# fnzhan/EMLight

Hardware: AMD Instinct MI355X
Metric: training images/sec (regression step: DenseNet-BC fwd + Sinkhorn loss + bwd + Adam) (higher is better)
Workload: dtype f32; 1 GPU; RegressionNetwork train step, BASELINE configs[1]; per_gpu_batch=64, global_batch=64, anchors=128, parallelism=single

## Files before the change

### emlight_amd/csrc/dense_bwd.hip

```cpp
#include "eml_common.h"
#include "eml_dropout.h"

#include <cstdint>
#include <cstdlib>
#include <type_traits>

namespace {

using eml::f32x4;
using eml::f4c;
using eml::mfma16;
using eml::shfl_xor_d;

constexpr int kTH = 8, kTW = 32, kHH = kTH + 2, kHW = kTW + 2;

constexpr int kPSG = 14;
constexpr int kBD = 512;
constexpr int kGRows = 2;
constexpr int kGPass = kHH / kGRows;

template <bool FUSE, bool WIDE, bool DROP = false>
__global__ __launch_bounds__(kBD, 2) void conv3x3_bwd_data_kernel(
    const float* __restrict__ G, int ldg, int c0, const float* __restrict__ W2, const float* __restrict__ Z,
    const float* __restrict__ zmean, const float* __restrict__ zistd, float* __restrict__ DZ, int B, int H, int W,
// ... 1221 lines not shown
          const float4 is = *reinterpret_cast<const float4*>(istd + k4);
          float l1[4] = {0.f, 0.f, 0.f, 0.f}, l2[4] = {0.f, 0.f, 0.f, 0.f};
#pragma unroll
          for (int m = 0; m < 4; ++m) {
            if (p0 + 16 * m + r < P) {
              const float da[4] = {acc[m][n][0], acc[m][n][1], acc[m][n][2], acc[m][n][3]};
              constexpr int NSUB = POOL ? 4 : 1;
#pragma unroll
              for (int sub = 0; sub < NSUB; ++sub) {
                const size_t pi = pin[m] + (sub >> 1) * (size_t)Win + (sub & 1);
                const float4 xv = *reinterpret_cast<const float4*>(X + pi * ldx + k4);
                float4* gp = reinterpret_cast<float4*>(Gd + pi * ldg + k4);
                float4 g = accumulate ? *gp : make_float4(0.f, 0.f, 0.f, 0.f);
                const float f = POOL ? 0.25f : 1.0f;
                const float d0 = (fmaf(xv.x, sk.x, tk.x) > 0.f) ? f * da[0] : 0.f;
                const float d1 = (fmaf(xv.y, sk.y, tk.y) > 0.f) ? f * da[1] : 0.f;
                const float d2 = (fmaf(xv.z, sk.z, tk.z) > 0.f) ? f * da[2] : 0.f;
                const float d3 = (fmaf(xv.w, sk.w, tk.w) > 0.f) ? f * da[3] : 0.f;
                g.x = fmaf(sk.x, d0, g.x);
                g.y = fmaf(sk.y, d1, g.y);
                g.z = fmaf(sk.z, d2, g.z);
                g.w = fmaf(sk.w, d3, g.w);
                *gp = g;
                l1[0] += d0;
                l1[1] += d1;
                l1[2] += d2;
                l1[3] += d3;
                l2[0] = fmaf(d0, (xv.x - mu.x) * is.x, l2[0]);
                l2[1] = fmaf(d1, (xv.y - mu.y) * is.y, l2[1]);
                l2[2] = fmaf(d2, (xv.z - mu.z) * is.z, l2[2]);
                l2[3] = fmaf(d3, (xv.w - mu.w) * is.w, l2[3]);
              }
            }
          }
#pragma unroll
          for (int g = 0; g < 4; ++g) {
            l1[g] = eml::row16_sum(l1[g]);
            l2[g] = eml::row16_sum(l2[g]);
            if (r == 0) {
              my[2 * (k4 + g)] += (double)l1[g];
              my[2 * (k4 + g) + 1] += (double)l2[g];
            }
          }
        }
      }
    }
  }
  __syncthreads();
  for (int e = tid; e < Kp * 2; e += 256)
    partials[(size_t)blockIdx.x * Kp * 2 + e] =
        (sacc[e] + sacc[(size_t)Kp * 2 + e]) + (sacc[(size_t)2 * Kp * 2 + e] + sacc[(size_t)3 * Kp * 2 + e]);
}

template <int MT, int NCH, bool ACC , bool MASKED = false, int NJO = 0>
__global__ __launch_bounds__(256, 2) void transition_bwd_data_kernel(
    const float* __restrict__ DY, int ld_dy, const float* __restrict__ Zr, int ld_z, const float* __restrict__ cA,
    const float* __restrict__ cB, const float* __restrict__ cC, int Ko, const float* __restrict__ Wd,
    const float* __restrict__ X, int ldx, const float* __restrict__ scale1, const float* __restrict__ shift1,
    const float* __restrict__ mean, const float* __restrict__ istd, int P, int Hin, int Win, int Kp,
    float* __restrict__ Gd, int ldg, double* __restrict__ partials ,
    const unsigned short* __restrict__ mask16) {
  extern __shared__ __attribute__((aligned(16))) float smem[];
  double* sacc = reinterpret_cast<double*>(smem);
  float* vec_l = reinterpret_cast<float*>(sacc + (size_t)4 * Kp * 2);
  float* co_l = vec_l + 4 * Kp;
  float* stg = co_l + 3 * Ko + (size_t)(threadIdx.x >> 6) * 16 * 36;
  const int tid = threadIdx.x, lane = tid & 63, wave = tid >> 6;
  const int r = lane & 15, kk = lane >> 4;
  for (int e = tid; e < 4 * Kp * 2; e += 256) sacc[e] = 0.0;
  for (int e = tid; e < Kp; e += 256) {
    vec_l[e] = scale1[e];
    vec_l[Kp + e] = shift1[e];
    vec_l[2 * Kp + e] = MASKED ? 0.f : mean[e];
    vec_l[3 * Kp + e] = MASKED ? 0.f : istd[e];
  }
  for (int e = tid; e < Ko; e += 256) {
    co_l[e] = cA[e];
    co_l[Ko + e] = cB[e];
    co_l[2 * Ko + e] = cC[e];
  }
  __syncthreads();
  double* my = sacc + (size_t)wave * Kp * 2;
  const int nnt = Kp >> 4, njo = Ko >> 4;
  constexpr int TP = 64 * MT;
  const int ntiles = (P + TP - 1) / TP;
  const int Wo = Win >> 1, Ho = Hin >> 1;

  for (int tile = blockIdx.x; tile < ntiles; tile += gridDim.x) {
    const int p0 = tile * TP + wave * 16 * MT;
    long prow[MT];
    size_t pin[MT];
    bool pv[MT];
#pragma unroll
    for (int m = 0; m < MT; ++m) {
      pv[m] = p0 + 16 * m + r < P;
      prow[m] = min(p0 + 16 * m + r, P - 1);
      const int b = (int)(prow[m] / (Ho * Wo)), rem = (int)(prow[m] - (long)b * (Ho * Wo));
      const int oy = rem / Wo, ox = rem - oy * Wo;
      pin[m] = (size_t)(b * Hin + 2 * oy) * Win + 2 * ox;
    }
    size_t pinx[MT][2];
    bool pvx[MT][2];
    if constexpr (MASKED && !ACC) {
#pragma unroll
      for (int m = 0; m < MT; ++m)
#pragma unroll
        for (int h = 0; h < 2; ++h) {
// ... 89 lines not shown
            dz[m].y = fmaf(a4.y, ry[m].y, fmaf(b4.y, rz[m].y, c4.y));
            dz[m].z = fmaf(a4.z, ry[m].z, fmaf(b4.z, rz[m].z, c4.z));
            dz[m].w = fmaf(a4.w, ry[m].w, fmaf(b4.w, rz[m].w, c4.w));
          }
          group_step(jo, dz);
        }
      }
      if constexpr (MASKED && !ACC) {
        float l1n[NCH][4];
        float4 skn[NCH];
#pragma unroll
        for (int n = 0; n < NCH; ++n) {
          skn[n] = *reinterpret_cast<const float4*>(vec_l + 16 * min(nt0 + n, nnt - 1) + 4 * kk);
#pragma unroll
          for (int g = 0; g < 4; ++g) l1n[n][g] = 0.f;
        }
        const int piece = lane & 7;
        const bool col_ok = nt0 + (piece >> 2) < nnt;
#pragma unroll
        for (int m = 0; m < MT; ++m) {
#pragma unroll
          for (int sub = 0; sub < 4; ++sub) {
#pragma unroll
            for (int n = 0; n < NCH; ++n) {
              const unsigned b = pv[m] ? mk[m][n] >> (4 * sub) : 0u;
              const float d0 = (b & 1u) ? 0.25f * acc[m][n][0] : 0.f, d1 = (b & 2u) ? 0.25f * acc[m][n][1] : 0.f;
              const float d2 = (b & 4u) ? 0.25f * acc[m][n][2] : 0.f, d3 = (b & 8u) ? 0.25f * acc[m][n][3] : 0.f;
              *reinterpret_cast<f32x4*>(stg + r * 36 + 16 * n + 4 * kk) = f32x4{skn[n].x * d0, skn[n].y * d1, skn[n].z * d2, skn[n].w * d3};
              if (nt0 + n < nnt) {
                l1n[n][0] += d0;
                l1n[n][1] += d1;
                l1n[n][2] += d2;
                l1n[n][3] += d3;
              }
            }
            __builtin_amdgcn_fence(__ATOMIC_RELEASE, "wavefront");
            __builtin_amdgcn_wave_barrier();
            __builtin_amdgcn_fence(__ATOMIC_ACQUIRE, "wavefront");
            const size_t suboff = ((size_t)(sub >> 1) * Win + (sub & 1)) * (size_t)ldg + 16 * nt0 + 4 * piece;
#pragma unroll
            for (int h = 0; h < 2; ++h) {
              const f32x4 v = *reinterpret_cast<const f32x4*>(stg + ((lane >> 3) + 8 * h) * 36 + 4 * piece);
              if (pvx[m][h] && col_ok) *reinterpret_cast<f32x4*>(Gd + pinx[m][h] * ldg + suboff) = v;
            }
            __builtin_amdgcn_fence(__ATOMIC_RELEASE, "wavefront");
            __builtin_amdgcn_wave_barrier();
            __builtin_amdgcn_fence(__ATOMIC_ACQUIRE, "wavefront");
          }
        }
#pragma unroll
        for (int n = 0; n < NCH; ++n) {
          if (nt0 + n < nnt) {
            const int k4 = 16 * (nt0 + n) + 4 * kk;
#pragma unroll
            for (int g = 0; g < 4; ++g) {
              const float t1 = eml::row16_sum(l1n[n][g]);
              if (r == 0) my[2 * (k4 + g)] += (double)t1;
            }
          }
        }
      } else {
#pragma unroll
      for (int n = 0; n < NCH; ++n) {
        const int nt = nt0 + n;
        if (nt < nnt) {
          const int k4 = 16 * nt + 4 * kk;
          const float4 sk = *reinterpret_cast<const float4*>(vec_l + k4);
          const float4 tk = *reinterpret_cast<const float4*>(vec_l + Kp + k4);
          const float4 mu = *reinterpret_cast<const float4*>(vec_l + 2 * Kp + k4);
          const float4 is = *reinterpret_cast<const float4*>(vec_l + 3 * Kp + k4);
          float l1[4] = {0.f, 0.f, 0.f, 0.f}, l2[4] = {0.f, 0.f, 0.f, 0.f};
#pragma unroll
          for (int m = 0; m < MT; ++m) {
            const float da0 = 0.25f * acc[m][n][0], da1 = 0.25f * acc[m][n][1];
            const float da2 = 0.25f * acc[m][n][2], da3 = 0.25f * acc[m][n][3];
#pragma unroll
            for (int sub = 0; sub < 4; ++sub) {
              float4 g = make_float4(0.f, 0.f, 0.f, 0.f);
              if constexpr (ACC) g = gs[m][n][sub];
              float d0, d1, d2, d3;
              float4 x = make_float4(0.f, 0.f, 0.f, 0.f);
              if constexpr (MASKED) {
                const unsigned b = pv[m] ? mk[m][n] >> (4 * sub) : 0u;
                d0 = (b & 1u) ? da0 : 0.f;
                d1 = (b & 2u) ? da1 : 0.f;
                d2 = (b & 4u) ? da2 : 0.f;
                d3 = (b & 8u) ? da3 : 0.f;
              } else {
                x = xv[m][n][sub];
                d0 = (pv[m] && fmaf(x.x, sk.x, tk.x) > 0.f) ? da0 : 0.f;
                d1 = (pv[m] && fmaf(x.y, sk.y, tk.y) > 0.f) ? da1 : 0.f;
                d2 = (pv[m] && fmaf(x.z, sk.z, tk.z) > 0.f) ? da2 : 0.f;
                d3 = (pv[m] && fmaf(x.w, sk.w, tk.w) > 0.f) ? da3 : 0.f;
              }
              g.x = fmaf(sk.x, d0, g.x);
              g.y = fmaf(sk.y, d1, g.y);
              g.z = fmaf(sk.z, d2, g.z);
              g.w = fmaf(sk.w, d3, g.w);
              if (pv[m]) {
                const size_t pi = pin[m] + (sub >> 1) * (size_t)Win + (sub & 1);
                *reinterpret_cast<float4*>(Gd + pi * ldg + k4) = g;
              }
              l1[0] += d0;
              l1[1] += d1;
              l1[2] += d2;
              l1[3] += d3;
              if constexpr (!MASKED) {
                l2[0] = fmaf(d0, (x.x - mu.x) * is.x, l2[0]);
                l2[1] = fmaf(d1, (x.y - mu.y) * is.y, l2[1]);
                l2[2] = fmaf(d2, (x.z - mu.z) * is.z, l2[2]);
                l2[3] = fmaf(d3, (x.w - mu.w) * is.w, l2[3]);
              }
            }
          }
#pragma unroll
          for (int g = 0; g < 4; ++g) {
            l1[g] = eml::row16_sum(l1[g]);
            if constexpr (!MASKED) l2[g] = eml::row16_sum(l2[g]);
            if (r == 0) {
              my[2 * (k4 + g)] += (double)l1[g];
              if constexpr (!MASKED) my[2 * (k4 + g) + 1] += (double)l2[g];
            }
          }
        }
      }
      }
    }
  }
  __syncthreads();
  for (int e = tid; e < Kp * 2; e += 256)
    partials[(size_t)blockIdx.x * Kp * 2 + e] =
        (sacc[e] + sacc[(size_t)Kp * 2 + e]) + (sacc[(size_t)2 * Kp * 2 + e] + sacc[(size_t)3 * Kp * 2 + e]);
}

struct BwdLayer {
  const float* DZ;
  const float* Zr;
  const float* cA;
  const float* cB;
  const float* cC;
  const float* Wd;
  const float* scale1;
  const float* shift1;
  double* partials;
  int Kp;
};

template <int NL, int MT , bool RAW = false ,
          bool MASKED = false, bool TOP = false>
__global__ __launch_bounds__(256, 2) void conv1x1_bwd_data_multi_kernel(BwdLayer L0, BwdLayer L1,
                                                                        const float* __restrict__ X, int ldx,
                                                                        const float* __restrict__ mean,
                                                                        const float* __restrict__ istd, int P,
                                                                        int k_lo, int k_hi, float* __restrict__ Gd,
                                                                        int ldg, int KpMax,
                                                                        const unsigned long long* __restrict__ M0,
                                                                        const unsigned long long* __restrict__ M1,
                                                                        float* __restrict__ Top) {
  extern __shared__ __attribute__((aligned(16))) float smem[];
  double* sacc = reinterpret_cast<double*>(smem);
  float* vec_l = reinterpret_cast<float*>(sacc + (size_t)NL * 4 * KpMax * 2);
  const int tid = threadIdx.x, lane = tid & 63, wave = tid >> 6;
  const int r = lane & 15, kk = lane >> 4;
  const BwdLayer Ls[2] = {L0, L1};
  for (int e = tid; e < NL * 4 * KpMax * 2; e += 256) sacc[e] = 0.0;
  for (int e = tid; e < KpMax; e += 256) {
    vec_l[e] = MASKED ? 0.f : mean[e];
    vec_l[KpMax + e] = MASKED ? 0.f : istd[e];
#pragma unroll
    for (int j = 0; j < NL; ++j) {
      vec_l[(2 + 2 * j) * KpMax + e] = e < Ls[j].Kp ? Ls[j].scale1[e] : 0.f;
      vec_l[(3 + 2 * j) * KpMax + e] = e < Ls[j].Kp ? Ls[j].shift1[e] : 0.f;
    }
  }
  __syncthreads();
  constexpr int TP = 64 * MT;
  const int ntiles = (P + TP - 1) / TP;
  const int nt_lo = k_lo >> 4, nt_hi = (k_hi + 15) >> 4;
  constexpr int NCH = 2;

  float4 wq[2][3][NCH];
  auto load_w = [&](int j, int nt0, float4 (&dst)[3][NCH]) {
    const int nnt = Ls[j].Kp >> 4;
#pragma unroll
    for (int jo = 0; jo < 3; ++jo)
#pragma unroll
      for (int n = 0; n < NCH; ++n) {
        const int nt = min(nt0 + n, nnt - 1);
        dst[jo][n] = *reinterpret_cast<const float4*>(Ls[j].Wd + ((((size_t)nt * 3 + jo) * 4 + kk) * 16 + r) * 4);
      }
  };
  load_w(0, nt_lo, wq[0]);
  int wsel = 0;

  for (int tile = blockIdx.x; tile < ntiles; tile += gridDim.x) {
    const int p0 = tile * TP + wave * 16 * MT;
    long prow[MT];
    bool pv[MT];
#pragma unroll
    for (int m = 0; m < MT; ++m) {
      pv[m] = p0 + 16 * m + r < P;
      prow[m] = min(p0 + 16 * m + r, P - 1);
    }
    unsigned long long pvb[MT];
#pragma unroll
    for (int m = 0; m < MT; ++m) pvb[m] = MASKED ? __ballot(pv[m]) : 0ull;
    float4 dz[NL][3][MT];
#pragma unroll
    for (int j = 0; j < NL; ++j)
#pragma unroll
      for (int jo = 0; jo < 3; ++jo) {
        const int ch = 16 * jo + 4 * kk;
        if constexpr (RAW) {
#pragma unroll
          for (int m = 0; m < MT; ++m) dz[j][jo][m] = *reinterpret_cast<const float4*>(Ls[j].DZ + prow[m] * 48 + ch);
        } else {
          const float4 a4 = *reinterpret_cast<const float4*>(Ls[j].cA + ch);
          const float4 b4 = *reinterpret_cast<const float4*>(Ls[j].cB + ch);
          const float4 c4 = *reinterpret_cast<const float4*>(Ls[j].cC + ch);
#pragma unroll
          for (int m = 0; m < MT; ++m) {
            const float4 dy = *reinterpret_cast<const float4*>(Ls[j].DZ + prow[m] * 48 + ch);
            const float4 zr = *reinterpret_cast<const float4*>(Ls[j].Zr + prow[m] * 48 + ch);
            dz[j][jo][m].x = fmaf(a4.x, dy.x, fmaf(b4.x, zr.x, c4.x));
            dz[j][jo][m].y = fmaf(a4.y, dy.y, fmaf(b4.y, zr.y, c4.y));
            dz[j][jo][m].z = fmaf(a4.z, dy.z, fmaf(b4.z, zr.z, c4.z));
            dz[j][jo][m].w = fmaf(a4.w, dy.w, fmaf(b4.w, zr.w, c4.w));
          }
        }
      }
    for (int nt0 = nt_lo; nt0 < nt_hi; nt0 += NCH) {
      float4 gs[MT][NCH], xv[MT][NCH];
#pragma unroll
      for (int n = 0; n < NCH; ++n) {
        const int k4 = 16 * min(nt0 + n, nt_hi - 1) + 4 * kk;
        const int k4l = (k4 + 3 >= k_lo && k4 < k_hi) ? k4 : (k_lo & ~3);
#pragma unroll
        for (int m = 0; m < MT; ++m) {
          gs[m][n] = *reinterpret_cast<const float4*>(Gd + prow[m] * ldg + k4l);
          if constexpr (!MASKED) xv[m][n] = *reinterpret_cast<const float4*>(X + prow[m] * ldx + k4l);
        }
      }
      const int nt_next = nt0 + NCH < nt_hi ? nt0 + NCH : nt_lo;
#pragma unroll
      for (int j = 0; j < NL; ++j) {
        const int nnt = Ls[j].Kp >> 4;
        unsigned long long mk[MT][NCH][4];
        if constexpr (MASKED) {
          const unsigned long long* __restrict__ Mj = j == 0 ? M0 : M1;
#pragma unroll
          for (int m = 0; m < MT; ++m)
#pragma unroll
            for (int n = 0; n < NCH; ++n) {
              const size_t wi =
                  ((size_t)__builtin_amdgcn_readfirstlane((p0 >> 4) + m) * nnt + min(nt0 + n, nnt - 1)) * 4;
#pragma unroll
              for (int g = 0; g < 4; ++g) mk[m][n][g] = Mj[wi + g];
            }
        }
        const int cur = NL == 2 ? j : wsel;
        if (j + 1 < NL)
          load_w(j + 1, nt0, wq[cur ^ 1]);
        else
          load_w(0, nt_next, wq[cur ^ 1]);
        __builtin_amdgcn_sched_barrier(0);
        f32x4 acc[MT][NCH];
#pragma unroll
        for (int m = 0; m < MT; ++m)
#pragma unroll
          for (int n = 0; n < NCH; ++n) acc[m][n] = f32x4{0.f, 0.f, 0.f, 0.f};
#pragma unroll
        for (int jo = 0; jo < 3; ++jo)
#pragma unroll
          for (int t = 0; t < 4; ++t)
#pragma unroll
            for (int n = 0; n < NCH; ++n)
#pragma unroll
              for (int m = 0; m < MT; ++m) acc[m][n] = mfma16(f4c(wq[cur][jo][n], t), f4c(dz[j][jo][m], t), acc[m][n]);
        if (NL == 1) wsel ^= 1;
        double* my = sacc + ((size_t)(j * 4 + wave) * KpMax) * 2;
#pragma unroll
        for (int n = 0; n < NCH; ++n) {
          const int nt = nt0 + n;
          if (nt < nnt && nt < nt_hi) {
            const int k4 = 16 * nt + 4 * kk;
            const float4 mu = *reinterpret_cast<const float4*>(vec_l + k4);
            const float4 is = *reinterpret_cast<const float4*>(vec_l + KpMax + k4);
            const float4 sk = *reinterpret_cast<const float4*>(vec_l + (2 + 2 * j) * KpMax + k4);
            const float4 tk = *reinterpret_cast<const float4*>(vec_l + (3 + 2 * j) * KpMax + k4);
            const bool in0 = k4 + 0 >= k_lo && k4 + 0 < k_hi, in1 = k4 + 1 >= k_lo && k4 + 1 < k_hi;
            const bool in2 = k4 + 2 >= k_lo && k4 + 2 < k_hi, in3 = k4 + 3 >= k_lo && k4 + 3 < k_hi;
            unsigned long long inb[4] = {0ull, 0ull, 0ull, 0ull};
            if constexpr (MASKED) {
              inb[0] = __ballot(in0);
              inb[1] = __ballot(in1);
              inb[2] = __ballot(in2);
              inb[3] = __ballot(in3);
            }
            float l1[4] = {0.f, 0.f, 0.f, 0.f}, l2[4] = {0.f, 0.f, 0.f, 0.f};
#pragma unroll
            for (int m = 0; m < MT; ++m) {
              float d0, d1, d2, d3;
              if constexpr (MASKED) {
                d0 = __builtin_amdgcn_inverse_ballot_w64(mk[m][n][0] & pvb[m] & inb[0]) ? acc[m][n][0] : 0.f;
                d1 = __builtin_amdgcn_inverse_ballot_w64(mk[m][n][1] & pvb[m] & inb[1]) ? acc[m][n][1] : 0.f;
                d2 = __builtin_amdgcn_inverse_ballot_w64(mk[m][n][2] & pvb[m] & inb[2]) ? acc[m][n][2] : 0.f;
                d3 = __builtin_amdgcn_inverse_ballot_w64(mk[m][n][3] & pvb[m] & inb[3]) ? acc[m][n][3] : 0.f;
              } else {
                const float4 x = xv[m][n];
                d0 = (pv[m] && in0 && fmaf(x.x, sk.x, tk.x) > 0.f) ? acc[m][n][0] : 0.f;
                d1 = (pv[m] && in1 && fmaf(x.y, sk.y, tk.y) > 0.f) ? acc[m][n][1] : 0.f;
                d2 = (pv[m] && in2 && fmaf(x.z, sk.z, tk.z) > 0.f) ? acc[m][n][2] : 0.f;
                d3 = (pv[m] && in3 && fmaf(x.w, sk.w, tk.w) > 0.f) ? acc[m][n][3] : 0.f;
                l2[0] = fmaf(d0, (x.x - mu.x) * is.x, l2[0]);
                l2[1] = fmaf(d1, (x.y - mu.y) * is.y, l2[1]);
                l2[2] = fmaf(d2, (x.z - mu.z) * is.z, l2[2]);
                l2[3] = fmaf(d3, (x.w - mu.w) * is.w, l2[3]);
              }
              gs[m][n].x = fmaf(sk.x, d0, gs[m][n].x);
              gs[m][n].y = fmaf(sk.y, d1, gs[m][n].y);
              gs[m][n].z = fmaf(sk.z, d2, gs[m][n].z);
              gs[m][n].w = fmaf(sk.w, d3, gs[m][n].w);
              l1[0] += d0;
              l1[1] += d1;
              l1[2] += d2;
              l1[3] += d3;
            }
#pragma unroll
            for (int g = 0; g < 4; ++g) {
              l1[g] = eml::row16_sum(l1[g]);
              if constexpr (!MASKED) l2[g] = eml::row16_sum(l2[g]);
              if (r == 0) {
                my[2 * (k4 + g)] += (double)l1[g];
                if constexpr (!MASKED) my[2 * (k4 + g) + 1] += (double)l2[g];
              }
            }
          }
        }
      }
#pragma unroll
      for (int n = 0; n < NCH; ++n) {
        const int nt = nt0 + n;
        if (nt < nt_hi) {
          const int k4 = 16 * nt + 4 * kk;
          const bool act = k4 + 3 >= k_lo && k4 < k_hi;
          if constexpr (TOP) {
            const int t = k4 - (k_hi - 24);
            float* cdst = Top + (t >= 12 ? (size_t)P * 12 + (t - 12) : (size_t)max(t, 0));
#pragma unroll
            for (int m = 0; m < MT; ++m) {
              float* dst = t >= 0 ? cdst + prow[m] * 12 : Gd + prow[m] * ldg + k4;
              if (pv[m] && act) *reinterpret_cast<float4*>(dst) = gs[m][n];
            }
          } else {
#pragma unroll
            for (int m = 0; m < MT; ++m) {
              if (pv[m] && act) *reinterpret_cast<float4*>(Gd + prow[m] * ldg + k4) = gs[m][n];
            }
          }
        }
      }
    }
  }
  __syncthreads();
#pragma unroll
  for (int j = 0; j < NL; ++j) {
    const int Kp = Ls[j].Kp;
    const double* base = sacc + (size_t)j * 4 * KpMax * 2;
    for (int e = tid; e < Kp * 2; e += 256)
      Ls[j].partials[(size_t)blockIdx.x * Kp * 2 + e] = (base[e] + base[(size_t)KpMax * 2 + e]) +
                                                        (base[(size_t)2 * KpMax * 2 + e] + base[(size_t)3 * KpMax * 2 + e]);
  }
}

template <int MT>
__global__ __launch_bounds__(256, 2) void conv1x1_bwd_narrow_kernel(
    const float* __restrict__ DZ, const float* __restrict__ W1 , int Cin, int k_lo,
    const float* __restrict__ X, int ldx, const float* __restrict__ scale1, const float* __restrict__ shift1,
    const float* __restrict__ mean, const float* __restrict__ istd, int P, const float* __restrict__ Gd, int ldg,
    float* __restrict__ N12, double* __restrict__ partials , int Kp) {
  __shared__ double red[4][12][2];
  const int tid = threadIdx.x, lane = tid & 63, wave = tid >> 6;
  const int r = lane & 15, kk = lane >> 4;
  float aw[3][4];
#pragma unroll
  for (int jo = 0; jo < 3; ++jo)
#pragma unroll
    for (int t = 0; t < 4; ++t) aw[jo][t] = r < 12 ? W1[(size_t)(16 * jo + 4 * kk + t) * Cin + k_lo + r] : 0.f;
  const bool cv = kk < 3;
  const int cq = k_lo + 4 * (cv ? kk : 2);
  float sk[4], tk[4], mu[4], is[4];
#pragma unroll
  for (int g = 0; g < 4; ++g) {
    sk[g] = scale1[cq + g];
    tk[g] = shift1[cq + g];
    mu[g] = mean[cq + g];
    is[g] = istd[cq + g];
  }
  double s1[4] = {0.0, 0.0, 0.0, 0.0}, s2[4] = {0.0, 0.0, 0.0, 0.0};
  constexpr int TP = 64 * MT;
  const int ntiles = (P + TP - 1) / TP;
  for (int tile = blockIdx.x; tile < ntiles; tile += gridDim.x) {
    const int p0 = tile * TP + wave * 16 * MT;
    size_t prow[MT];
    bool pv[MT];
    float4 dz[MT][3];
    float2 xa[MT], xb[MT], ga[MT], gb[MT];
#pragma unroll
    for (int m = 0; m < MT; ++m) {
      pv[m] = p0 + 16 * m + r < P;
// ... 738 lines not shown

extern "C" int eml_dense_conv1x1_bwd_weight_f32(const float* X, int ldx, long P, int Hin, int Win, int pool, int Kp,
                                                int Cin, const float* scale1, const float* shift1, const float* DY,
                                                int ld_dy, const float* Zr, int ld_z, const float* cA, const float* cB,
                                                const float* cC, int Cout, float* partial, float* dW, int grid,
                                                float* dz_out, const float* W1, int k_lo, const float* G, int ldg,
                                                float* N12, double* partials_n, eml_stream_t stream) {
  if (dz_out && (Cout != 48 || pool))
    return eml::fail(EML_EINVAL, "eml_dense_conv1x1_bwd_weight_f32: dz_out is for dense layers (Cout == 48, no pool)");
  if (N12 && (Cout != 48 || pool || !W1 || !G || !partials_n || k_lo < 0 || (k_lo & 1) || k_lo + 12 > Cin || (ldg & 1) ||
              (ldg != 12 && k_lo + 12 > ldg)))
    return eml::fail(EML_EINVAL, "eml_dense_conv1x1_bwd_weight_f32: fused narrow pass needs a dense layer, W1, G, partials_n "
                                 "and an even k_lo with k_lo + 12 <= Cin (k_lo=%d, Cin=%d)", k_lo, Cin);
  if (!X || !scale1 || !shift1 || !DY || !Zr || !cA || !cB || !cC || !partial || !dW || P < 1 || grid < 1 || Kp < 32 ||
      (Kp & 15) || Cin > Kp || Cout < 1)
    return eml::fail(EML_EINVAL, "eml_dense_conv1x1_bwd_weight_f32: bad arguments");
  const int nchunks = (Cout + 47) / 48;
  for (int ch = 0; ch < nchunks; ++ch) {
    const int n0 = ch * 48, nv = (Cout - n0 < 48) ? Cout - n0 : 48;
    int n_load = ((ld_dy < ld_z ? ld_dy : ld_z) - n0) & ~3;
    if (n_load > 48) n_load = 48;
    if (n_load < nv) return eml::fail(EML_EINVAL, "eml_dense_conv1x1_bwd_weight_f32: DY/Zr rows narrower than Cout");
    const NarrowArgs na{W1, G, N12, partials_n, Cin, k_lo, ldg};
    if (pool)
      hipLaunchKernelGGL((conv1x1_bwd_weight_kernel<true, false>), dim3(grid), dim3(256), 0, (hipStream_t)stream, X, ldx,
                         (int)P, Hin, Win, Kp, scale1, shift1, DY + n0, ld_dy, Zr + n0, ld_z, cA + n0, cB + n0, cC + n0,
                         nv, n_load, partial, nullptr, na);
    else if (N12)
      hipLaunchKernelGGL((conv1x1_bwd_weight_kernel<false, true>), dim3(grid), dim3(256), 0, (hipStream_t)stream, X, ldx,
                         (int)P, Hin, Win, Kp, scale1, shift1, DY + n0, ld_dy, Zr + n0, ld_z, cA + n0, cB + n0, cC + n0,
                         nv, n_load, partial, dz_out, na);
    else
      hipLaunchKernelGGL((conv1x1_bwd_weight_kernel<false, false>), dim3(grid), dim3(256), 0, (hipStream_t)stream, X, ldx,
                         (int)P, Hin, Win, Kp, scale1, shift1, DY + n0, ld_dy, Zr + n0, ld_z, cA + n0, cB + n0, cC + n0,
                         nv, n_load, partial, dz_out, na);
    int rc = eml::check_launch("eml_dense_conv1x1_bwd_weight_f32");
    if (rc) return rc;
    hipLaunchKernelGGL(reduce_rows_kernel, dim3((Cin * 48 + 63) / 64), dim3(256), 0, (hipStream_t)stream, partial,
                       grid, (size_t)Kp * 48, 0, Cin, nv, n0, dW);
    rc = eml::check_launch("eml_dense_conv1x1_bwd_weight_f32(reduce)");
    if (rc) return rc;
  }
  return EML_OK;
}

extern "C" int eml_dense_permute_w1_bwd_f32(const float* W, int Cout, int Cin, int Kp, int Ko, float* Wd,
                                            eml_stream_t stream) {
  if (!W || !Wd || Cout < 1 || Cin < 1 || Kp < Cin || (Kp & 15) || Ko < Cout || (Ko & 15))
    return eml::fail(EML_EINVAL, "eml_dense_permute_w1_bwd_f32: bad arguments");
  hipLaunchKernelGGL(permute_w1_bwd_kernel, dim3(64), dim3(256), 0, (hipStream_t)stream, W, Cout, Cin, Kp, Ko, Wd);
  return eml::check_launch("eml_dense_permute_w1_bwd_f32");
}

extern "C" int eml_dense_conv1x1_bwd_data_f32(const float* DY, int ld_dy, const float* Zr, int ld_z, const float* cA,
                                              const float* cB, const float* cC, int Ko, const float* Wd,
                                              const float* X, int ldx, const float* scale1, const float* shift1,
                                              const float* mean, const float* istd, long P, int Hin, int Win, int pool,
                                              int Kp, float* G, int ldg, int accumulate, double* partials, int grid,
                                              const unsigned short* relu_mask16, eml_stream_t stream) {
  if (!DY || !Zr || !cA || !cB || !cC || !Wd || (!relu_mask16 && (!X || !mean || !istd)) || !scale1 || !shift1 || !G ||
      !partials || P < 1 || grid < 1 || (Kp & 15) || (Ko & 15) || Ko > ld_dy || Ko > ld_z || (ld_dy & 3) || (ld_z & 3) ||
      (ldx & 3) || (ldg & 3) || (!relu_mask16 && Kp > ldx) || Kp > ldg)
    return eml::fail(EML_EINVAL, "eml_dense_conv1x1_bwd_data_f32: bad arguments");
  if (relu_mask16 && !(pool && Ko != 48))
    return eml::fail(EML_EINVAL, "eml_dense_conv1x1_bwd_data_f32: relu_mask16 is for the transition form (pool, Ko != 48)");
  const size_t lds = (size_t)4 * Kp * 2 * sizeof(double);
#define EML_LAUNCH_BWD_DATA(POOLV, RESV, NCHV)                                                                        \
  hipLaunchKernelGGL((conv1x1_bwd_data_kernel<POOLV, RESV, NCHV>), dim3(grid), dim3(256), lds, (hipStream_t)stream, DY, \
                     ld_dy, Zr, ld_z, cA, cB, cC, Ko, Wd, X, ldx, scale1, shift1, mean, istd, (int)P, Hin, Win, Kp, G, \
                     ldg, accumulate, partials)
  if (pool) {
    if (Ko == 48) {
      EML_LAUNCH_BWD_DATA(true, true, 4);
    } else {
      const size_t lds_t = lds + (size_t)(4 * Kp + 3 * Ko + 4 * 16 * 36) * sizeof(float);
#define EML_LAUNCH_TRANSITION(ACCV, MSKV)                                                                              \
  do {                                                                                                                \
    EML_ENSURE_LDS((&transition_bwd_data_kernel<2, 2, ACCV, MSKV>), lds_t);                                 \
    hipLaunchKernelGGL((transition_bwd_data_kernel<2, 2, ACCV, MSKV>), dim3(grid), dim3(256), lds_t,                   \
                       (hipStream_t)stream, DY, ld_dy, Zr, ld_z, cA, cB, cC, Ko, Wd, X, ldx, scale1, shift1, mean, istd, \
                       (int)P, Hin, Win, Kp, G, ldg, partials, relu_mask16);                                           \
  } while (0)
#define EML_LAUNCH_TRANSITION_RES(NJOV)                                                                                \
  do {                                                                                                                \
    EML_ENSURE_LDS((&transition_bwd_data_kernel<2, 2, false, true, NJOV>), lds_t);                                     \
    hipLaunchKernelGGL((transition_bwd_data_kernel<2, 2, false, true, NJOV>), dim3(grid), dim3(256), lds_t,            \
                       (hipStream_t)stream, DY, ld_dy, Zr, ld_z, cA, cB, cC, Ko, Wd, X, ldx, scale1, shift1, mean, istd, \
                       (int)P, Hin, Win, Kp, G, ldg, partials, relu_mask16);                                           \
  } while (0)
      if (relu_mask16 && !accumulate && Ko == 112) EML_LAUNCH_TRANSITION_RES(7);
      else if (relu_mask16 && !accumulate && Ko == 160) EML_LAUNCH_TRANSITION_RES(10);
      else if (relu_mask16 && !accumulate && Ko == 176) EML_LAUNCH_TRANSITION_RES(11);
      else if (relu_mask16) {
        if (accumulate) EML_LAUNCH_TRANSITION(true, true); else EML_LAUNCH_TRANSITION(false, true);
      } else {
        if (accumulate) EML_LAUNCH_TRANSITION(true, false); else EML_LAUNCH_TRANSITION(false, false);
      }
#undef EML_LAUNCH_TRANSITION
#undef EML_LAUNCH_TRANSITION_RES
    }
  } else {
    if (Ko == 48) EML_LAUNCH_BWD_DATA(false, true, 2); else EML_LAUNCH_BWD_DATA(false, false, 4);
  }
#undef EML_LAUNCH_BWD_DATA
  return eml::check_launch("eml_dense_conv1x1_bwd_data_f32");
}

namespace {
int launch_bwd_data_multi(int n_layers, const float* const* DZ, const float* const* Zr, const float* const* cA,
                          const float* const* cB, const float* const* cC, const float* const* Wd,
                          const float* const* scale1, const float* const* shift1, double* const* partials, const int* Kp,
                          const float* X, int ldx, const float* mean, const float* istd, long P, int k_lo, int k_hi,
                          float* G, int ldg, int grid, const unsigned long long* const* relu_masks, float* top,
                          eml_stream_t stream) {
  if (top && (n_layers != 2 || !relu_masks || Zr || k_lo != 0 || k_hi < 24 || (k_hi & 3) || P * 12 > 2147483647L))
    return eml::fail(EML_EINVAL, "eml_dense_conv1x1_bwd_data_multi_top_f32: the compact top-24 output needs two layers, "
                                 "relu_masks, materialised dz, k_lo == 0 and k_hi >= 24, a multiple of 4 (k_hi=%d)", k_hi);
  if (n_layers < 1 || n_layers > 2 || !DZ || !Wd || !scale1 || !shift1 || !partials ||
      !Kp || (!relu_masks && (!X || !mean || !istd)) || !G || P < 1 || grid < 1 || k_lo < 0 || k_hi <= k_lo ||
      (ldx & 3) || (ldg & 3))
    return eml::fail(EML_EINVAL, "eml_dense_conv1x1_bwd_data_multi_f32: bad arguments");
  const bool raw = Zr == nullptr;
  if (!raw && (!cA || !cB || !cC))
    return eml::fail(EML_EINVAL, "eml_dense_conv1x1_bwd_data_multi_f32: Zr given without cA/cB/cC");
  if (relu_masks && !raw)
    return eml::fail(EML_EINVAL, "eml_dense_conv1x1_bwd_data_multi_f32: relu_masks needs the materialised dz (Zr == NULL)");
  BwdLayer L[2];
  const unsigned long long* Mk[2] = {nullptr, nullptr};
  int kmax = 0;
  for (int j = 0; j < 2; ++j) {
    const int s = j < n_layers ? j : 0;
    const unsigned long long* mk = relu_masks ? relu_masks[s] : nullptr;
    Mk[j] = mk;
    L[j] = raw ? BwdLayer{DZ[s], nullptr, nullptr, nullptr, nullptr, Wd[s], scale1[s], shift1[s], partials[s], Kp[s]}
               : BwdLayer{DZ[s], Zr[s], cA[s], cB[s], cC[s], Wd[s], scale1[s], shift1[s], partials[s], Kp[s]};
    if (!DZ[s] || (!raw && !Zr[s]) || !Wd[s] || !partials[s] || (relu_masks && !mk) || (Kp[s] & 15) ||
        (!relu_masks && Kp[s] > ldx) || Kp[s] > ldg)
      return eml::fail(EML_EINVAL, "eml_dense_conv1x1_bwd_data_multi_f32: bad layer %d", s);
    if (Kp[s] > kmax) kmax = Kp[s];
  }
  if (((k_hi + 15) & ~15) > kmax) return eml::fail(EML_EINVAL, "eml_dense_conv1x1_bwd_data_multi_f32: range beyond Kp");
  const size_t lds = (size_t)n_layers * 4 * kmax * 2 * sizeof(double) + (size_t)(2 + 2 * n_layers) * kmax * sizeof(float);
  if (lds > 80 * 1024) return eml::fail(EML_EINVAL, "eml_dense_conv1x1_bwd_data_multi_f32: Kp=%d does not fit LDS", kmax);
#define EML_LAUNCH_MULTI(NLV, MTV, RAWV, MSKV)                                                                       \
  do {                                                                                                              \
    EML_ENSURE_LDS((&conv1x1_bwd_data_multi_kernel<NLV, MTV, RAWV, MSKV>), lds);                                 \
    hipLaunchKernelGGL((conv1x1_bwd_data_multi_kernel<NLV, MTV, RAWV, MSKV>), dim3(grid), dim3(256), lds,            \
                       (hipStream_t)stream, L[0], L[1], X, ldx, mean, istd, (int)P, k_lo, k_hi, G, ldg, kmax,        \
                       Mk[0], Mk[1], (float*)nullptr);                                                              \
  } while (0)
  if (n_layers == 1) {
    if (relu_masks) EML_LAUNCH_MULTI(1, 4, true, true);
    else if (raw) EML_LAUNCH_MULTI(1, 4, true, false);
    else EML_LAUNCH_MULTI(1, 4, false, false);
  } else if (top) {
    EML_ENSURE_LDS((&conv1x1_bwd_data_multi_kernel<2, 2, true, true, true>), lds);
    hipLaunchKernelGGL((conv1x1_bwd_data_multi_kernel<2, 2, true, true, true>), dim3(grid), dim3(256), lds,
                       (hipStream_t)stream, L[0], L[1], X, ldx, mean, istd, (int)P, k_lo, k_hi, G, ldg, kmax, Mk[0], Mk[1],
                       top);
  } else {
    if (relu_masks) EML_LAUNCH_MULTI(2, 2, true, true);
    else if (raw) EML_LAUNCH_MULTI(2, 2, true, false);
    else EML_LAUNCH_MULTI(2, 2, false, false);
  }
#undef EML_LAUNCH_MULTI
  return eml::check_launch("eml_dense_conv1x1_bwd_data_multi_f32");
}
}

extern "C" int eml_dense_conv1x1_bwd_data_multi_f32(int n_layers, const float* const* DZ, const float* const* Zr,
                                                    const float* const* cA, const float* const* cB,
                                                    const float* const* cC, const float* const* Wd,
                                                    const float* const* scale1, const float* const* shift1,
                                                    double* const* partials, const int* Kp, const float* X, int ldx,
                                                    const float* mean, const float* istd, long P, int k_lo, int k_hi,
                                                    float* G, int ldg, int grid,
                                                    const unsigned long long* const* relu_masks, eml_stream_t stream) {
  return launch_bwd_data_multi(n_layers, DZ, Zr, cA, cB, cC, Wd, scale1, shift1, partials, Kp, X, ldx, mean, istd, P, k_lo,
                               k_hi, G, ldg, grid, relu_masks, nullptr, stream);
}

extern "C" int eml_dense_conv1x1_bwd_data_multi_top_f32(const float* const* DZ, const float* const* Wd,
                                                        const float* const* scale1, const float* const* shift1,
                                                        double* const* partials, const int* Kp, long P, int k_hi,
                                                        float* G, int ldg, int grid,
                                                        const unsigned long long* const* relu_masks, float* top,
                                                        eml_stream_t stream) {
  if (!top) return eml::fail(EML_EINVAL, "eml_dense_conv1x1_bwd_data_multi_top_f32: top is NULL");
  return launch_bwd_data_multi(2, DZ, nullptr, nullptr, nullptr, nullptr, Wd, scale1, shift1, partials, Kp, nullptr, 0,
                               nullptr, nullptr, P, 0, k_hi, G, ldg, grid, relu_masks, top, stream);
}

extern "C" int eml_dense_conv1x1_bwd_narrow_f32(const float* DZ, const float* W1, int Cin, int k_lo, const float* X,
                                                int ldx, const float* scale1, const float* shift1, const float* mean,
                                                const float* istd, long P, const float* G, int ldg, float* N12,
                                                double* partials, int Kp, int grid, eml_stream_t stream) {
  if (!DZ || !W1 || !X || !scale1 || !shift1 || !mean || !istd || !G || !N12 || !partials || P < 1 || grid < 1 ||
      k_lo < 0 || (k_lo & 1) || k_lo + 12 > Cin || Cin > Kp || (ldx & 1) || (ldg & 1) || Kp > ldx || Kp > ldg)
    return eml::fail(EML_EINVAL, "eml_dense_conv1x1_bwd_narrow_f32: bad arguments");
  hipLaunchKernelGGL((conv1x1_bwd_narrow_kernel<4>), dim3(grid), dim3(256), 0, (hipStream_t)stream, DZ, W1, Cin, k_lo, X,
                     ldx, scale1, shift1, mean, istd, (int)P, G, ldg, N12, partials, Kp);
  return eml::check_launch("eml_dense_conv1x1_bwd_narrow_f32");
}

extern "C" int eml_dense_grad_materialize_f32(float* G, int ldg, const float* X, int ldx, const float* sB,
                                              const float* sC, int c0, int n, long P, eml_stream_t stream) {
  if (!G || !X || !sB || !sC || P < 1 || n < 2 || (n & 1) || (c0 & 1) || (ldg & 1) || (ldx & 1))
    return eml::fail(EML_EINVAL, "eml_dense_grad_materialize_f32: bad arguments");
  const size_t total = (size_t)P * (n >> 1);
  const int grid = (int)((total + 255) / 256 < 8192 ? (total + 255) / 256 : 8192);
  hipLaunchKernelGGL(grad_materialize_kernel, dim3(grid), dim3(256), 0, (hipStream_t)stream, G, ldg, X, ldx, sB, sC, c0,
                     n, (size_t)P);
  return eml::check_launch("eml_dense_grad_materialize_f32");
}

extern "C" int eml_dense_bn_bwd_stats_f32(const float* DY, int ld_dy, const float* raw, int ld_raw, const float* out,
                                          int ld_out, int relu, int C, long P, const float* mean, const float* istd,
                                          double* partials, int grid, eml_stream_t stream) {
// ... 95 lines not shown
```

Before: 569.5 images/s.

## Rework dgrad epilogue: packed DPP row reductions, LDS f64 atomics, 32-bit addressing

Adds an EPI path (on by default, disabled with EML_DGRAD_EPILOGUE=0) to the transition and multi 1x1 backward-data kernels. It reduces four BN-stat channels together with DPP moves and has lanes r<4 each add one channel into LDS with workgroup-scope f64 atomic adds, replacing four serial row16 reductions done by lane 0. It also switches store addressing to 32-bit offsets from a wave-uniform base, preloads scale vectors with scalar-forcing hints, and raises the min-blocks launch bound to 3 for masked EPI. The aim is fewer instructions and VGPRs in the epilogue and higher occupancy, at the cost of LDS atomic contention and possible spills.

```diff
diff --git a/emlight_amd/csrc/dense_bwd.hip b/emlight_amd/csrc/dense_bwd.hip
--- a/emlight_amd/csrc/dense_bwd.hip
+++ b/emlight_amd/csrc/dense_bwd.hip
@@ -1297,7 +1297,30 @@
         (sacc[e] + sacc[(size_t)Kp * 2 + e]) + (sacc[(size_t)2 * Kp * 2 + e] + sacc[(size_t)3 * Kp * 2 + e]);
 }
 
-template <int MT, int NCH, bool ACC , bool MASKED = false, int NJO = 0>
+__device__ __forceinline__ float row16_sum4_pick(const float (&v)[4], int r) {
+  float a = v[0], b = v[1], c = v[2], d = v[3];
+  a += eml::dpp_mov<0xB1>(a), b += eml::dpp_mov<0xB1>(b), c += eml::dpp_mov<0xB1>(c), d += eml::dpp_mov<0xB1>(d);
+  a += eml::dpp_mov<0x4E>(a), b += eml::dpp_mov<0x4E>(b), c += eml::dpp_mov<0x4E>(c), d += eml::dpp_mov<0x4E>(d);
+  a += eml::dpp_mov<0x141>(a), b += eml::dpp_mov<0x141>(b), c += eml::dpp_mov<0x141>(c), d += eml::dpp_mov<0x141>(d);
+  a += eml::dpp_mov<0x140>(a), b += eml::dpp_mov<0x140>(b), c += eml::dpp_mov<0x140>(c), d += eml::dpp_mov<0x140>(d);
+  const float ab = (r & 1) ? b : a, cd = (r & 1) ? d : c;
+  return (r & 2) ? cd : ab;
+}
+__device__ __forceinline__ void lds_add_f64(double* p, double v) {
+  (void)__hip_atomic_fetch_add(p, v, __ATOMIC_RELAXED, __HIP_MEMORY_SCOPE_WORKGROUP);
+}
+__device__ __forceinline__ int uniform_here(int v) {
+  v = __builtin_amdgcn_readfirstlane(v);
+  asm volatile("" : "+s"(v));
+  return v;
+}
+__device__ __forceinline__ double to_f64_here(float v) {
+  double d = (double)v;
+  asm volatile("" : "+v"(d));
+  return d;
+}
+
+template <int MT, int NCH, bool ACC , bool MASKED = false, int NJO = 0, bool EPI = true>
 __global__ __launch_bounds__(256, 2) void transition_bwd_data_kernel(
     const float* __restrict__ DY, int ld_dy, const float* __restrict__ Zr, int ld_z, const float* __restrict__ cA,
     const float* __restrict__ cB, const float* __restrict__ cC, int Ko, const float* __restrict__ Wd,
@@ -1493,10 +1516,15 @@
         for (int n = 0; n < NCH; ++n) {
           if (nt0 + n < nnt) {
             const int k4 = 16 * (nt0 + n) + 4 * kk;
+            if constexpr (EPI) {
+              const double t1 = to_f64_here(row16_sum4_pick(l1n[n], r));
+              if (r < 4) lds_add_f64(&my[2 * (k4 + r)], t1);
+            } else {
 #pragma unroll
             for (int g = 0; g < 4; ++g) {
               const float t1 = eml::row16_sum(l1n[n][g]);
               if (r == 0) my[2 * (k4 + g)] += (double)t1;
+            }
             }
           }
         }
@@ -1554,6 +1582,15 @@
               }
             }
           }
+          if constexpr (EPI) {
+            const double t1 = to_f64_here(row16_sum4_pick(l1, r));
+            double t2 = 0.0;
+            if constexpr (!MASKED) t2 = to_f64_here(row16_sum4_pick(l2, r));
+            if (r < 4) {
+              lds_add_f64(&my[2 * (k4 + r)], t1);
+              if constexpr (!MASKED) lds_add_f64(&my[2 * (k4 + r) + 1], t2);
+            }
+          } else {
 #pragma unroll
           for (int g = 0; g < 4; ++g) {
             l1[g] = eml::row16_sum(l1[g]);
@@ -1562,6 +1599,7 @@
               my[2 * (k4 + g)] += (double)l1[g];
               if constexpr (!MASKED) my[2 * (k4 + g) + 1] += (double)l2[g];
             }
+          }
           }
         }
       }
@@ -1588,8 +1626,8 @@
 };
 
 template <int NL, int MT , bool RAW = false ,
-          bool MASKED = false, bool TOP = false>
-__global__ __launch_bounds__(256, 2) void conv1x1_bwd_data_multi_kernel(BwdLayer L0, BwdLayer L1,
+          bool MASKED = false, bool TOP = false, bool EPI = true>
+__global__ __launch_bounds__(256, (MASKED && EPI) ? 3 : 2) void conv1x1_bwd_data_multi_kernel(BwdLayer L0, BwdLayer L1,
                                                                         const float* __restrict__ X, int ldx,
                                                                         const float* __restrict__ mean,
                                                                         const float* __restrict__ istd, int P,
@@ -1617,6 +1655,7 @@
   __syncthreads();
   constexpr int TP = 64 * MT;
   const int ntiles = (P + TP - 1) / TP;
+  const int stat_lane = wave * KpMax * 2 + 2 * (4 * kk + (r & 3));
   const int nt_lo = k_lo >> 4, nt_hi = (k_hi + 15) >> 4;
   constexpr int NCH = 2;
 
@@ -1628,7 +1667,7 @@
 #pragma unroll
       for (int n = 0; n < NCH; ++n) {
         const int nt = min(nt0 + n, nnt - 1);
-        dst[jo][n] = *reinterpret_cast<const float4*>(Ls[j].Wd + ((((size_t)nt * 3 + jo) * 4 + kk) * 16 + r) * 4);
+        dst[jo][n] = *reinterpret_cast<const float4*>(Ls[j].Wd + ((((unsigned)nt * 3 + jo) * 4 + kk) * 16 + r) * 4);
       }
   };
   load_w(0, nt_lo, wq[0]);
@@ -1643,6 +1682,11 @@
       pv[m] = p0 + 16 * m + r < P;
       prow[m] = min(p0 + 16 * m + r, P - 1);
     }
+    const int pb = __builtin_amdgcn_readfirstlane(min(p0, P - 1));
+    float* __restrict__ Gt = Gd + (size_t)pb * ldg;
+    unsigned grow[MT];
+#pragma unroll
+    for (int m = 0; m < MT; ++m) grow[m] = (unsigned)((int)prow[m] - pb) * (unsigned)ldg;
     unsigned long long pvb[MT];
 #pragma unroll
     for (int m = 0; m < MT; ++m) pvb[m] = MASKED ? __ballot(pv[m]) : 0ull;
@@ -1678,7 +1722,7 @@
         const int k4l = (k4 + 3 >= k_lo && k4 < k_hi) ? k4 : (k_lo & ~3);
 #pragma unroll
         for (int m = 0; m < MT; ++m) {
-          gs[m][n] = *reinterpret_cast<const float4*>(Gd + prow[m] * ldg + k4l);
+          gs[m][n] = *reinterpret_cast<const float4*>(Gt + (grow[m] + (unsigned)k4l));
           if constexpr (!MASKED) xv[m][n] = *reinterpret_cast<const float4*>(X + prow[m] * ldx + k4l);
         }
       }
@@ -1718,6 +1762,23 @@
             for (int n = 0; n < NCH; ++n)
 #pragma unroll
               for (int m = 0; m < MT; ++m) acc[m][n] = mfma16(f4c(wq[cur][jo][n], t), f4c(dz[j][jo][m], t), acc[m][n]);
+        float4 skq[NCH];
+        if constexpr (EPI) {
+          __builtin_amdgcn_sched_barrier(0);
+#pragma unroll
+          for (int n = 0; n < NCH; ++n)
+            skq[n] = *reinterpret_cast<const float4*>(
+                vec_l + (uniform_here((2 + 2 * j) * KpMax + 16 * min(nt0 + n, nt_hi - 1)) + 4 * kk));
+          if constexpr (MASKED) {
+#pragma unroll
+            for (int m = 0; m < MT; ++m)
+#pragma unroll
+              for (int n = 0; n < NCH; ++n)
+                asm volatile("" ::"s"(mk[m][n][0]), "s"(mk[m][n][1]), "s"(mk[m][n][2]), "s"(mk[m][n][3]));
+          }
+#pragma unroll
+          for (int n = 0; n < NCH; ++n) asm volatile("" ::"v"(skq[n].x), "v"(skq[n].y), "v"(skq[n].z), "v"(skq[n].w));
+        }
         if (NL == 1) wsel ^= 1;
         double* my = sacc + ((size_t)(j * 4 + wave) * KpMax) * 2;
 #pragma unroll
@@ -1727,7 +1788,9 @@
             const int k4 = 16 * nt + 4 * kk;
             const float4 mu = *reinterpret_cast<const float4*>(vec_l + k4);
             const float4 is = *reinterpret_cast<const float4*>(vec_l + KpMax + k4);
-            const float4 sk = *reinterpret_cast<const float4*>(vec_l + (2 + 2 * j) * KpMax + k4);
+            float4 sk;
+            if constexpr (EPI) sk = skq[n];
+            else sk = *reinterpret_cast<const float4*>(vec_l + (2 + 2 * j) * KpMax + k4);
             const float4 tk = *reinterpret_cast<const float4*>(vec_l + (3 + 2 * j) * KpMax + k4);
             const bool in0 = k4 + 0 >= k_lo && k4 + 0 < k_hi, in1 = k4 + 1 >= k_lo && k4 + 1 < k_hi;
             const bool in2 = k4 + 2 >= k_lo && k4 + 2 < k_hi, in3 = k4 + 3 >= k_lo && k4 + 3 < k_hi;
@@ -1767,6 +1830,16 @@
               l1[2] += d2;
               l1[3] += d3;
             }
+            if constexpr (EPI) {
+              const double t1 = to_f64_here(row16_sum4_pick(l1, r));
+              double t2 = 0.0;
+              if constexpr (!MASKED) t2 = to_f64_here(row16_sum4_pick(l2, r));
+              double* acc_r = sacc + (uniform_here(j * 4 * KpMax * 2 + 32 * nt) + stat_lane);
+              if (r < 4) {
+                lds_add_f64(acc_r, t1);
+                if constexpr (!MASKED) lds_add_f64(acc_r + 1, t2);
+              }
+            } else {
 #pragma unroll
             for (int g = 0; g < 4; ++g) {
               l1[g] = eml::row16_sum(l1[g]);
@@ -1776,6 +1849,7 @@
                 if constexpr (!MASKED) my[2 * (k4 + g) + 1] += (double)l2[g];
               }
             }
+            }
           }
         }
       }
@@ -1787,16 +1861,23 @@
           const bool act = k4 + 3 >= k_lo && k4 < k_hi;
           if constexpr (TOP) {
             const int t = k4 - (k_hi - 24);
-            float* cdst = Top + (t >= 12 ? (size_t)P * 12 + (t - 12) : (size_t)max(t, 0));
-#pragma unroll
-            for (int m = 0; m < MT; ++m) {
-              float* dst = t >= 0 ? cdst + prow[m] * 12 : Gd + prow[m] * ldg + k4;
-              if (pv[m] && act) *reinterpret_cast<float4*>(dst) = gs[m][n];
+            if (t >= 0) {
+              const unsigned c0 = t >= 12 ? (unsigned)P * 12u + (unsigned)(t - 12) : (unsigned)t;
+#pragma unroll
+              for (int m = 0; m < MT; ++m) {
+                unsigned pr = (unsigned)prow[m];
+                asm volatile("" : "+v"(pr));
+                if (pv[m] && act) *reinterpret_cast<float4*>(Top + (c0 + pr * 12u)) = gs[m][n];
+              }
+            } else {
+#pragma unroll
+              for (int m = 0; m < MT; ++m)
+                if (pv[m] && act) *reinterpret_cast<float4*>(Gt + (grow[m] + (unsigned)k4)) = gs[m][n];
             }
           } else {
 #pragma unroll
             for (int m = 0; m < MT; ++m) {
-              if (pv[m] && act) *reinterpret_cast<float4*>(Gd + prow[m] * ldg + k4) = gs[m][n];
+              if (pv[m] && act) *reinterpret_cast<float4*>(Gt + (grow[m] + (unsigned)k4)) = gs[m][n];
             }
           }
         }
@@ -2641,6 +2722,11 @@
   return eml::check_launch("eml_dense_permute_w1_bwd_f32");
 }
 
+static bool dgrad_epilogue_env() {
+  static const bool on = [] { const char* v = getenv("EML_DGRAD_EPILOGUE"); return !(v && v[0] == '0'); }();
+  return on;
+}
+
 extern "C" int eml_dense_conv1x1_bwd_data_f32(const float* DY, int ld_dy, const float* Zr, int ld_z, const float* cA,
                                               const float* cB, const float* cC, int Ko, const float* Wd,
                                               const float* X, int ldx, const float* scale1, const float* shift1,
@@ -2663,19 +2749,21 @@
       EML_LAUNCH_BWD_DATA(true, true, 4);
     } else {
       const size_t lds_t = lds + (size_t)(4 * Kp + 3 * Ko + 4 * 16 * 36) * sizeof(float);
-#define EML_LAUNCH_TRANSITION(ACCV, MSKV)                                                                              \
+      const bool epi = dgrad_epilogue_env();
+#define EML_LAUNCH_TRANSITION_(ACCV, MSKV, NJOV, EPIV)                                                                 \
   do {                                                                                                                \
-    EML_ENSURE_LDS((&transition_bwd_data_kernel<2, 2, ACCV, MSKV>), lds_t);                                 \
-    hipLaunchKernelGGL((transition_bwd_data_kernel<2, 2, ACCV, MSKV>), dim3(grid), dim3(256), lds_t,                   \
+    EML_ENSURE_LDS((&transition_bwd_data_kernel<2, 2, ACCV, MSKV, NJOV, EPIV>), lds_t);                                \
+    hipLaunchKernelGGL((transition_bwd_data_kernel<2, 2, ACCV, MSKV, NJOV, EPIV>), dim3(grid), dim3(256), lds_t,       \
                        (hipStream_t)stream, DY, ld_dy, Zr, ld_z, cA, cB, cC, Ko, Wd, X, ldx, scale1, shift1, mean, istd, \
                        (int)P, Hin, Win, Kp, G, ldg, partials, relu_mask16);                                           \
   } while (0)
+#define EML_LAUNCH_TRANSITION(ACCV, MSKV)                                                                              \
+  do {                                                                                                                \
+    if (epi) EML_LAUNCH_TRANSITION_(ACCV, MSKV, 0, true); else EML_LAUNCH_TRANSITION_(ACCV, MSKV, 0, false);           \
+  } while (0)
 #define EML_LAUNCH_TRANSITION_RES(NJOV)                                                                                \
   do {                                                                                                                \
-    EML_ENSURE_LDS((&transition_bwd_data_kernel<2, 2, false, true, NJOV>), lds_t);                                     \
-    hipLaunchKernelGGL((transition_bwd_data_kernel<2, 2, false, true, NJOV>), dim3(grid), dim3(256), lds_t,            \
-                       (hipStream_t)stream, DY, ld_dy, Zr, ld_z, cA, cB, cC, Ko, Wd, X, ldx, scale1, shift1, mean, istd, \
-                       (int)P, Hin, Win, Kp, G, ldg, partials, relu_mask16);                                           \
+    if (epi) EML_LAUNCH_TRANSITION_(false, true, NJOV, true); else EML_LAUNCH_TRANSITION_(false, true, NJOV, false);   \
   } while (0)
       if (relu_mask16 && !accumulate && Ko == 112) EML_LAUNCH_TRANSITION_RES(7);
       else if (relu_mask16 && !accumulate && Ko == 160) EML_LAUNCH_TRANSITION_RES(10);
@@ -2687,6 +2775,7 @@
       }
 #undef EML_LAUNCH_TRANSITION
 #undef EML_LAUNCH_TRANSITION_RES
+#undef EML_LAUNCH_TRANSITION_
     }
   } else {
     if (Ko == 48) EML_LAUNCH_BWD_DATA(false, true, 2); else EML_LAUNCH_BWD_DATA(false, false, 4);
@@ -2731,28 +2820,32 @@
   if (((k_hi + 15) & ~15) > kmax) return eml::fail(EML_EINVAL, "eml_dense_conv1x1_bwd_data_multi_f32: range beyond Kp");
   const size_t lds = (size_t)n_layers * 4 * kmax * 2 * sizeof(double) + (size_t)(2 + 2 * n_layers) * kmax * sizeof(float);
   if (lds > 80 * 1024) return eml::fail(EML_EINVAL, "eml_dense_conv1x1_bwd_data_multi_f32: Kp=%d does not fit LDS", kmax);
+  const bool epi = dgrad_epilogue_env();
+#define EML_LAUNCH_MULTI_(NLV, MTV, RAWV, MSKV, TOPV, EPIV)                                                          \
+  do {                                                                                                              \
+    EML_ENSURE_LDS((&conv1x1_bwd_data_multi_kernel<NLV, MTV, RAWV, MSKV, TOPV, EPIV>), lds);                         \
+    hipLaunchKernelGGL((conv1x1_bwd_data_multi_kernel<NLV, MTV, RAWV, MSKV, TOPV, EPIV>), dim3(grid), dim3(256),     \
+                       lds, (hipStream_t)stream, L[0], L[1], X, ldx, mean, istd, (int)P, k_lo, k_hi, G, ldg, kmax,   \
+                       Mk[0], Mk[1], TOPV ? top : (float*)nullptr);                                                 \
+  } while (0)
 #define EML_LAUNCH_MULTI(NLV, MTV, RAWV, MSKV)                                                                       \
   do {                                                                                                              \
-    EML_ENSURE_LDS((&conv1x1_bwd_data_multi_kernel<NLV, MTV, RAWV, MSKV>), lds);                                 \
-    hipLaunchKernelGGL((conv1x1_bwd_data_multi_kernel<NLV, MTV, RAWV, MSKV>), dim3(grid), dim3(256), lds,            \
-                       (hipStream_t)stream, L[0], L[1], X, ldx, mean, istd, (int)P, k_lo, k_hi, G, ldg, kmax,        \
-                       Mk[0], Mk[1], (float*)nullptr);                                                              \
+    if (epi) EML_LAUNCH_MULTI_(NLV, MTV, RAWV, MSKV, false, true);                                                  \
+    else EML_LAUNCH_MULTI_(NLV, MTV, RAWV, MSKV, false, false);                                                     \
   } while (0)
   if (n_layers == 1) {
     if (relu_masks) EML_LAUNCH_MULTI(1, 4, true, true);
     else if (raw) EML_LAUNCH_MULTI(1, 4, true, false);
     else EML_LAUNCH_MULTI(1, 4, false, false);
   } else if (top) {
-    EML_ENSURE_LDS((&conv1x1_bwd_data_multi_kernel<2, 2, true, true, true>), lds);
-    hipLaunchKernelGGL((conv1x1_bwd_data_multi_kernel<2, 2, true, true, true>), dim3(grid), dim3(256), lds,
-                       (hipStream_t)stream, L[0], L[1], X, ldx, mean, istd, (int)P, k_lo, k_hi, G, ldg, kmax, Mk[0], Mk[1],
-                       top);
+    if (epi) EML_LAUNCH_MULTI_(2, 2, true, true, true, true); else EML_LAUNCH_MULTI_(2, 2, true, true, true, false);
   } else {
     if (relu_masks) EML_LAUNCH_MULTI(2, 2, true, true);
     else if (raw) EML_LAUNCH_MULTI(2, 2, true, false);
     else EML_LAUNCH_MULTI(2, 2, false, false);
   }
 #undef EML_LAUNCH_MULTI
+#undef EML_LAUNCH_MULTI_
   return eml::check_launch("eml_dense_conv1x1_bwd_data_multi_f32");
 }
 }
```

Result: no change. 573.1 images/s (median of 6 runs) (+0.6%).
